# Tomeu7/AO-MARL

Hardware: AMD Instinct MI355X
Metric: env steps/sec (AO frames/sec) (higher is better)
Workload: dtype f32

## Files before the change

ao_marl_amd/csrc/aomarl_capi_composites.hip:

```cpp
const char *aomarl_frame_kernel_name(aomarl_ctx *c) {
  if (!c || !c->fw_variant[0]) return "";
  snprintf(c->fw_name, sizeof(c->fw_name), "k_frame_wave<%d, %d, %s, %s, %s, %s>", c->fw_variant[0], c->fw_variant[1],
           c->fw_variant[2] ? "true" : "false", c->fw_variant[3] ? "true" : "false",
           c->fw_variant[4] ? "true" : "false", c->fw_variant[5] ? "true" : "false");
  return c->fw_name;
}

int aomarl_frame_kernel_time(aomarl_ctx *c, double *total_ms, int *launches) {
  if (!c || !total_ms || !launches) return fail("frame_kernel_time: null argument");
  double tot = 0.0;
  int n = 0;
  for (size_t i = 0; i + 1 < c->fw_ev_used; i += 2) {
    float ms = 0.f;
    HIPCHK(hipEventSynchronize(c->fw_ev[i + 1]));
    HIPCHK(hipEventElapsedTime(&ms, c->fw_ev[i], c->fw_ev[i + 1]));
    tot += ms; n++;
  }
  { const int rrc = fw_ev_rewind(c); if (rrc) return rrc; }
  *total_ms = tot; *launches = n;
  return 0;
}

int aomarl_frame_fused_available(aomarl_ctx *c) {
  return c && c->sys.fused_ok && !c->force_unfused_frame ? 1 : 0;
}

static int frame_fused_impl(aomarl_ctx *c, aomarl_state *st, int b, int n, int flags, void *stream, int slot);

int aomarl_frame_fused(aomarl_ctx *c, aomarl_state *st, int b, int n, int flags, void *stream) {
  return frame_fused_impl(c, st, b, n, flags, stream, -1);
}

static int frame_fused_impl(aomarl_ctx *c, aomarl_state *st, int b, int n, int flags, void *stream, int slot) {
  int rc = check_range(c, st, b, n);
  if (rc) return rc;
  if (slot < 0) {
    rc = atmos_wait_pending(c, stream);
    if (rc) return rc;
    rc = psf_wait_pending(c, stream);
    if (rc) return rc;
  }
  if (!c->sys.fused_ok) return fail("frame_fused: geometry not eligible (see aomarl_frame_fused_available)");
  if (flags & (AOMARL_IMG_FROM_PHASE_BUFFER | AOMARL_IMG_NO_ATMOS | AOMARL_IMG_NO_DMS))
    return fail("frame_fused: FROM_PHASE_BUFFER / NO_ATMOS / NO_DMS are not supported here");
  const bool noise = (flags & AOMARL_IMG_NOISE) && c->sys.noise >= 0.f;
  const bool cube = flags & AOMARL_IMG_WRITE_BINCUBE;
  const bool otf = flags & AOMARL_IMG_DM_FROM_VOLTAGE;
  const int cog = ((flags & AOMARL_IMG_COG) ? 1 : 0) | (c->fused_debug << 8);
  if (otf && !c->sys.otf_ok) return fail("frame_fused: DM_FROM_VOLTAGE needs a separable stack-array lattice (see aomarl_dm_from_voltage_available)");
  if (cube && !st->bincube) return fail("frame_fused: WRITE_BINCUBE needs st->bincube");
  if (!cube && !(cog & 1)) return fail("frame_fused: nothing to produce (neither bincube nor slopes)");
  if (n == 0) return 0;
  hipStream_t s = (hipStream_t)stream;
  Work w = work_layout(c, st->nenv);
  const int W = 2 * c->sys.hw;
  float *TR = st->work + w.TR + (size_t)b * c->sys.pupdiam * W * 2;
  float *TP = st->work + w.TPART + (size_t)b * w.nblk * 4;
  float *PEND = st->work + w.PEND + (size_t)b * (W * W + 4);
  DevState ds = dev_state(st);
  if (w.nblk != c->sys.ntiles) return fail("frame_fused: internal stripe count mismatch");
  const int nb = otf ? c->sys.otf_nb : 1;
  const bool hp = c->dft_mode < 0 ? g_precision != 0 : c->dft_mode == 1;
  const bool qf = FW_QF && otf && !hp && !noise && !cube;
  const bool dma = FW_DMA && otf && (hp || FW_DMA_F32);
  const size_t smm = sizeof(float) * ((qf ? 0 : 2 * 128) + (otf ? 4 * 4 * nb * c->sys.otf_latw : 0)) + FW_SLOT_BYTES(dma) +
                     (dma ? 4 * FWD_WAVE(c->nlayers == 1 ? 1 : 3) : 128) +
                     (qf ? 4 * 16 * (size_t)c->sys.ntiles : 0);
  static const long lds_pad_env = [] { const char *e = getenv("AOMARL_FW_LDS_PAD"); return e ? atol(e) : -1L; }();
  size_t lds_pad = 0;
  if (qf && slot >= 0 && smm >= 40 * 1024) {
    const size_t two_per_cu = (160 * 1024) / 3 + 64;
    lds_pad = lds_pad_env >= 0 ? (size_t)lds_pad_env : (smm < two_per_cu ? (two_per_cu - smm + 63) / 64 * 64 : 0);
    if (smm + lds_pad > 64 * 1024) lds_pad = 0;
  }
  dim3 grid((n + 3) / 4, c->sys.ntiles), blk(256);
#define FW(NL, NB, OTF, NZ, WC, HP) hipExtLaunchKernelGGL((k_frame_wave<NL, NB, OTF, NZ, WC, HP>), grid, blk, smm + lds_pad, s, ev_start, ev_done, 0, c->sys, ds, b, n, cog, TR, TP, w.nblk)
#define FW_H(NL, NB, OTF, NZ, WC) do { if (hp) FW(NL, NB, OTF, NZ, WC, true); else FW(NL, NB, OTF, NZ, WC, false); } while (0)
#define FW_NC(NL, NB, OTF)                                                                     \
  do {                                                                                          \
    if (noise) { if (cube) FW_H(NL, NB, OTF, true, true); else FW_H(NL, NB, OTF, true, false); }     \
    else { if (cube) FW_H(NL, NB, OTF, false, true); else FW_H(NL, NB, OTF, false, false); }         \
  } while (0)
#define FW_L(NL)                                                          \
  do {                                                                    \
    if (!otf) FW_NC(NL, 1, false);                                        \
    else if (nb == 1) FW_NC(NL, 1, true);                                 \
    else FW_NC(NL, 2, true);                                              \
  } while (0)
  const bool timed = !c->capturing && c->time_fw && c->fw_ev_used + 2 <= c->fw_ev.size();
  hipEvent_t ev_start = nullptr, ev_done = nullptr;
  if (c->prefetch_atmos) {
    rc = side_stream(c);
    if (rc) return rc;
    ev_done = slot < 0 ? c->ev_frame : c->pipe.ev_done[slot];
  }
  if (timed) { ev_start = c->fw_ev[c->fw_ev_used]; ev_done = c->fw_ev[c->fw_ev_used + 1]; c->fw_ev_used += 2; }
  hipEvent_t ev_mark = nullptr;
  if (c->capturing) { ev_mark = ev_done; ev_start = nullptr; ev_done = nullptr; }
  if (c->nlayers == 1) FW_L(1); else FW_L(3);
  if (ev_mark) { HIPCHK(hipEventRecord(ev_mark, s)); ev_done = ev_mark; }
  c->frame_marked = false;
  c->fw_variant[0] = c->nlayers == 1 ? 1 : 3; c->fw_variant[1] = otf ? nb : 1; c->fw_variant[2] = otf;
  c->fw_variant[3] = noise; c->fw_variant[4] = cube; c->fw_variant[5] = hp;
  g_arith[hp ? AR_FRAME_SPLIT : AR_FRAME_F32]++;
#undef FW_L
#undef FW_NC
#undef FW_H
#undef FW
  LAUNCHCHK();
  if (slot >= 0) {
    c->pipe.ev_done_cur[slot] = ev_done;
    HIPCHK(hipStreamWaitEvent(c->psf_stream, ev_done, 0));
    if (!c->pipe.cmd_covers_commit)
      HIPCHK(hipStreamWaitEvent(c->psf_stream, c->pipe.ev_commit, 0));
    hipExtLaunchKernelGGL(k_target_finish_mfma, dim3(n), dim3(256), 0, c->psf_stream, nullptr, c->pipe.ev_psf[slot], 0, c->sys, TR,
                          TP, w.nblk, PEND, st->frame + b);
    LAUNCHCHK();
    c->pipe.psf_out[slot] = true;
    return 0;
  }
  if (c->prefetch_atmos) {
    c->ev_frame_cur = ev_done; c->frame_marked = true;
    c->side_joined = false;
    HIPCHK(hipStreamWaitEvent(c->psf_stream, ev_done, 0));
    hipExtLaunchKernelGGL(k_target_finish_mfma, dim3(n), dim3(256), 0, c->psf_stream, nullptr, c->capturing ? nullptr : c->ev_psf, 0,
                          c->sys, TR, TP, w.nblk, PEND, st->frame + b);
    LAUNCHCHK();
    if (c->capturing) HIPCHK(hipEventRecord(c->ev_psf, c->psf_stream));
    c->psf_side = true;
    return 0;
  }
  hipLaunchKernelGGL(k_target_finish_mfma, dim3(n), dim3(256), 0, s, c->sys, TR, TP, w.nblk, PEND, st->frame + b);
  LAUNCHCHK();
  return 0;
}

int aomarl_materialize_dm_shape(aomarl_ctx *c, aomarl_state *st, int b, int n, void *stream) {
  int rc = check_range(c, st, b, n);
  if (rc) return rc;
  if (n == 0) return 0;
  return dm_shape_impl(c, st, b, n, nullptr, false, stream);
}

int aomarl_next_part_one(aomarl_ctx *c, aomarl_state *st, int b, int n, float *accumx, float *accumy,
                         int image_flags, void *stream) {
  int rc = aomarl_move_atmos(c, st, b, n, accumx, accumy, stream);
  if (rc) return rc;
  int fl = (image_flags | AOMARL_IMG_COG | AOMARL_IMG_NOISE) & ~(AOMARL_IMG_NO_ATMOS | AOMARL_IMG_NO_DMS);
  const bool defer = c->defer_dm_shape && aomarl_dm_from_voltage_available(c);
  if (aomarl_frame_fused_available(c) && !(fl & AOMARL_IMG_FROM_PHASE_BUFFER)) {
// ... 146 lines not shown
```

ao_marl_amd/csrc/aomarl_kernels.hip:

```cpp
#include "aomarl_host.h"
#include "aomarl_gemm_p.h"
#include <type_traits>

#define WAVE 64

typedef unsigned u32x4 __attribute__((ext_vector_type(4)));

__device__ __forceinline__ hx2 cvt_h2(float a, float b) {
  return __builtin_bit_cast(hx2, __builtin_amdgcn_cvt_pkrtz(a, b));
}
__device__ __forceinline__ float sub_lo(hx2 h, float a) {
  float r;
  asm("v_fma_mix_f32 %0, %1, -1.0, %2 op_sel_hi:[1,0,0]" : "=v"(r) : "v"(h), "v"(a));
  return r;
}
__device__ __forceinline__ float sub_hi(hx2 h, float a) {
  float r;
  asm("v_fma_mix_f32 %0, %1, -1.0, %2 op_sel:[1,0,0] op_sel_hi:[1,0,0]" : "=v"(r) : "v"(h), "v"(a));
  return r;
}

struct __attribute__((packed, aligned(4))) f4u { float v[4]; };
__device__ __forceinline__ void add4(float acc[4], const float *p) {
  const f4u t = *reinterpret_cast<const f4u *>(p);
// ... 1447 lines not shown
    }
  }
}

struct SpotQf { f32x2 Ml, Mh, Sl, Sh; };

__device__ __forceinline__ SpotQf spot_qf_consts(int lane, const float2 *sTw ) {
  const int q = lane >> 4, c = lane & 15;
  float m[4], sv[4];
#pragma unroll
  for (int s = 0; s < 4; s++) {
    const int d = c - (4 * q + s);
    float a = 0.f, b = 0.f;
    for (int j = 0; j < 16; j++) {
      const float2 w = sTw[((2 * j + 1) * d) & 127];
      a += w.x;
      b = fmaf(0.5f + (float)(j >> 1), w.y, b);
    }
    m[s] = (d != 0 && (d & 1) == 0) ? 0.f : 2.f * a;
    sv[s] = 2.f * b;
  }
  SpotQf k;
  k.Ml = f32x2{m[0], m[1]}; k.Mh = f32x2{m[2], m[3]};
  k.Sl = f32x2{sv[0], sv[1]}; k.Sh = f32x2{sv[2], sv[3]};
  return k;
}

__global__ __launch_bounds__(128) void k_fill_qf_tab(float *__restrict__ tab) {
  __shared__ float2 sTw[128];
  const int tid = threadIdx.x;
  float sn, cs;
  sincospif((float)tid * (1.0f / 64.0f), &sn, &cs);
  sTw[tid] = make_float2(cs, sn);
  __syncthreads();
  if (tid < 64) {
    const SpotQf k = spot_qf_consts(tid, sTw);
    float *o = tab + 8 * tid;
    o[0] = k.Ml.x; o[1] = k.Ml.y; o[2] = k.Mh.x; o[3] = k.Mh.y;
    o[4] = k.Sl.x; o[5] = k.Sl.y; o[6] = k.Sh.x; o[7] = k.Sh.y;
  }
}

typedef unsigned u32x2 __attribute__((ext_vector_type(2)));
__device__ __forceinline__ float swap32_add(float a, float b) {
  const u32x2 t = __builtin_amdgcn_permlane32_swap(__float_as_uint(a), __float_as_uint(b), false, false);
  return __uint_as_float(t[0]) + __uint_as_float(t[1]);
}
__device__ __forceinline__ float swap16_add(float a, float b) {
  const u32x2 t = __builtin_amdgcn_permlane16_swap(__float_as_uint(a), __float_as_uint(b), false, false);
  return __uint_as_float(t[0]) + __uint_as_float(t[1]);
}
__device__ __forceinline__ float spot_qf_moments(const SpotQf &K, const float (&er)[4], const float (&ei)[4], const f32x4 z4) {
  const float Mc[4] = {K.Ml.x, K.Ml.y, K.Mh.x, K.Mh.y}, Sc[4] = {K.Sl.x, K.Sl.y, K.Sh.x, K.Sh.y};
  f32x4 Wr = z4, Wi = z4, V = z4;
#pragma unroll
  for (int s = 0; s < 4; s++) {
    Wr = mfma16(Mc[s], er[s], Wr);
    Wi = mfma16(Mc[s], ei[s], Wi);
    V = mfma16(Sc[s], er[s], V);
  }
  f32x4 G1 = z4, G2 = z4, G3 = z4;
#pragma unroll
  for (int s = 0; s < 4; s++) {
    G1 = mfma16(er[s], Wr[s], G1);
    G2 = mfma16(ei[s], Wr[s], G2);
    G3 = mfma16(ei[s], V[s], G3);
    G1 = mfma16(ei[s], Wi[s], G1);
  }
  PK_GUARD_MFMA();
  f32x2 p0 = pk_mul(pk_lo(G1), K.Ml);
  f32x2 px = pk_mul(pk_lo(G3), K.Ml);
  f32x2 py = pk_mul(pk_lo(G2), K.Sl);
  pk_acc_fma(p0, pk_hi(G1), K.Mh);
  pk_acc_fma(px, pk_hi(G3), K.Mh);
  pk_acc_fma(py, pk_hi(G2), K.Sh);
  const float s0 = p0.x + p0.y, tx = px.x + px.y, ty = py.x + py.y;
  float z = swap16_add(swap32_add(s0, tx), swap32_add(ty, p0.y));
  z += dpp_f<0xB1>(z);
  z += dpp_f<0x4E>(z);
  z += dpp_f<0x141>(z);
  z += dpp_f<0x140>(z);
  return z;
}
__device__ __forceinline__ void qf_slopes(const DevSys &sys, float s0, float tx, float ty, float &sx, float &sy) {
  if (s0 > 0.f) {
    const float inv = 2.f * __builtin_amdgcn_rcpf(s0);
    sx = (fmaf(tx, inv, 7.5f) - sys.cog_offset) * sys.cog_scale;
    sy = (fmaf(-ty, inv, 7.5f) - sys.cog_offset) * sys.cog_scale;
  } else {
    sx = 0.f; sy = 0.f;
  }
}

template <bool NOISE, bool WRITE_CUBE>
__device__ __forceinline__ void spot_finish_v(const DevSys &sys, const DevState &st, int e, int i,
                                              int lane, const float (&v)[2][2][2], int do_cog,
                                              float flux_i) {
  const int q = lane >> 4, c = lane & 15;
  const bool owner = (c & 1) == 0;
  float tot = 0.f;
#pragma unroll
  for (int sy = 0; sy < 2; sy++)
#pragma unroll
    for (int sx = 0; sx < 2; sx++)
#pragma unroll
      for (int h = 0; h < 2; h++) tot += v[sy][sx][h];
  const int Xp = 8 + (c >> 1), Xm = 7 - (c >> 1);
  if (!NOISE && !WRITE_CUBE) {
    const float A0 = (v[0][0][0] + v[0][0][1]) + (v[1][0][0] + v[1][0][1]);
    const float A1 = (v[0][1][0] + v[0][1][1]) + (v[1][1][0] + v[1][1][1]);
    float sx_ = (float)Xp * A0;
    sx_ = fmaf((float)Xm, A1, sx_);
    float sy_ = (float)(8 + 2 * q) * (v[0][0][0] + v[0][1][0]);
    sy_ = fmaf((float)(9 + 2 * q), v[0][0][1] + v[0][1][1], sy_);
    sy_ = fmaf((float)(7 - 2 * q), v[1][0][0] + v[1][1][0], sy_);
    sy_ = fmaf((float)(6 - 2 * q), v[1][0][1] + v[1][1][1], sy_);
    tot = wave_sum_last(A0 + A1);
    sx_ = wave_sum_last(sx_);
    sy_ = wave_sum_last(sy_);
    if (do_cog && lane == 63) {
      float *sl = st.slopes + (long long)e * sys.nslope;
      if (tot > 0.f) {
        const float inv = __builtin_amdgcn_rcpf(tot);
        sl[i] = (sx_ * inv - sys.cog_offset) * sys.cog_scale;
        sl[sys.nvalid + i] = (sy_ * inv - sys.cog_offset) * sys.cog_scale;
      } else {
        sl[i] = 0.f;
        sl[sys.nvalid + i] = 0.f;
      }
    }
    (void)flux_i;
    return;
  }
  tot = wave_sum(owner ? tot : 0.f);
  const float g = tot > 0.f ? sys.nphot * flux_i / tot : 0.f;
  float s0 = 0.f, sx = 0.f, sy = 0.f;
  if (NOISE) {
    const int hh = c & 1;
    const uint32_t sd = st.seeds[e], fr = st.frame[e];
#pragma unroll
    for (int ty_ = 0; ty_ < 2; ty_++)
#pragma unroll
      for (int tx_ = 0; tx_ < 2; tx_++) {
        const int Y = ty_ ? 7 - (2 * q + hh) : 8 + 2 * q + hh, X = tx_ ? Xm : Xp;
        const uint32_t idx = (uint32_t)i * 256u + (uint32_t)(Y * 16 + X);
        const float val = sh_noise((hh ? v[ty_][tx_][1] : v[ty_][tx_][0]) * g, sys.noise, sd, fr, idx);
        if (WRITE_CUBE) st.bincube[((long long)e * sys.nvalid + i) * 256 + Y * 16 + X] = val;
        s0 += val;
        sx += val * (float)X;
        sy += val * (float)Y;
      }
  } else {
#pragma unroll
    for (int ty_ = 0; ty_ < 2; ty_++)
#pragma unroll
      for (int tx_ = 0; tx_ < 2; tx_++)
#pragma unroll
        for (int h = 0; h < 2; h++) {
          const int Y = ty_ ? 7 - (2 * q + h) : 8 + 2 * q + h, X = tx_ ? Xm : Xp;
          const float val = v[ty_][tx_][h] * g;
          if (WRITE_CUBE && owner)
            st.bincube[((long long)e * sys.nvalid + i) * 256 + Y * 16 + X] = val;
          s0 += val;
          sx += val * (float)X;
          sy += val * (float)Y;
        }
// ... 349 lines not shown
          }
      tot = wave_sum(owner ? tot : 0.f);
      sx_ = wave_sum(owner ? sx_ : 0.f);
      sy_ = wave_sum(owner ? sy_ : 0.f);
      if (do_cog && lane == 0) {
        const float inv = tot > 0.f ? 1.0f / tot : 0.f;
        sl[i] = tot > 0.f ? (sx_ * inv - sys.cog_offset) * sys.cog_scale : 0.f;
        sl[sys.nvalid + i] = tot > 0.f ? (sy_ * inv - sys.cog_offset) * sys.cog_scale : 0.f;
      }
    } else {
      tot = wave_sum(owner ? tot : 0.f);
      const float g = tot > 0.f ? sys.nphot * flux_cur / tot : 0.f;
      float s0 = 0.f, sx = 0.f, sy = 0.f;
      if (NOISE) {
        const int hh = c & 1;
        const uint32_t sd = st.seeds[e], fr = st.frame[e];
#pragma unroll
        for (int ty_ = 0; ty_ < 2; ty_++)
#pragma unroll
          for (int tx_ = 0; tx_ < 2; tx_++) {
            const int Y = ty_ ? 7 - (2 * q + hh) : 8 + 2 * q + hh, X = tx_ ? Xm : Xp;
            const uint32_t idx = (uint32_t)i * 256u + (uint32_t)(Y * 16 + X);
            const float val = sh_noise((hh ? v[ty_][tx_][1] : v[ty_][tx_][0]) * g, sys.noise, sd, fr, idx);
            if (WRITE_CUBE) st.bincube[((long long)e * sys.nvalid + i) * 256 + Y * 16 + X] = val;
            s0 += val;
            sx += val * (float)X;
            sy += val * (float)Y;
          }
      } else {
#pragma unroll
        for (int ty_ = 0; ty_ < 2; ty_++)
#pragma unroll
          for (int tx_ = 0; tx_ < 2; tx_++)
#pragma unroll
            for (int h = 0; h < 2; h++) {
              const int Y = ty_ ? 7 - (2 * q + h) : 8 + 2 * q + h, X = tx_ ? Xm : Xp;
              const float val = v[ty_][tx_][h] * g;
              if (WRITE_CUBE && owner)
                st.bincube[((long long)e * sys.nvalid + i) * 256 + Y * 16 + X] = val;
              s0 += val;
              sx += val * (float)X;
              sy += val * (float)Y;
            }
      }
      if (do_cog) {
        s0 = wave_sum((NOISE || owner) ? s0 : 0.f);
        sx = wave_sum((NOISE || owner) ? sx : 0.f);
        sy = wave_sum((NOISE || owner) ? sy : 0.f);
        if (lane == 0) {
          sl[i] = s0 != 0.f ? (sx / s0 - sys.cog_offset) * sys.cog_scale : 0.f;
          sl[sys.nvalid + i] = s0 != 0.f ? (sy / s0 - sys.cog_offset) * sys.cog_scale : 0.f;
        }
      }
    }
    flux_cur = flux_next;
    __builtin_amdgcn_wave_barrier();
  }
}

#define FW_LD 20
#define FW_LIT 0x10000
#define FW_FULL 0x20000
#define FW_SUB 0x40000
__device__ __forceinline__ float sci_rev(float ph, float inv_lambda) { return ph * inv_lambda; }

typedef const int __attribute__((address_space(4))) *const_int_p;
typedef const float __attribute__((address_space(4))) *const_float_p;

template <int NL, bool OTF>
struct FrameRaw {
  float L[NL][4];
  float P[OTF ? 1 : 4], T[8];
  unsigned mrow;
  float F;
  f4u SH;
  float4 CS;
};

template <int NL, int NB, bool OTF, bool NOISE, bool WRITE_CUBE, bool HP>
#ifndef FW_WAVES
#define FW_WAVES 3
#endif
#ifndef FW_QF
#define FW_QF 1
#endif
#ifndef FW_DMA
#define FW_DMA 1
#endif
#ifndef FW_DEPTH
#define FW_DEPTH 2
#endif
#ifndef FW_DMA_F32
#define FW_DMA_F32 1
#endif
#ifndef FW_SLOTS1
#define FW_SLOTS1 0
#endif
#define FW_SLOT_BYTES(dma) ((dma) ? (FW_SLOTS1 ? 2 * 3 * 1024 : 16384) : 16384)
#define FWD_BLK 1152
#define FWD_IMG (2 * 1024 + 128)
#define FWD_WAVE(nl) ((nl) * FWD_IMG)
__global__ __launch_bounds__(256) __attribute__((amdgpu_waves_per_eu(FW_WAVES, FW_WAVES)))
void k_frame_wave(DevSys sys, DevState st, int env_begin,
                                                    int env_count, int do_cog,
                                                    float *__restrict__ TR,
                                                    float *__restrict__ TPART, int nblk) {
  extern __shared__ float smem[];
  const int pd = sys.pupdiam, ntl = sys.ntiles;
  const int tid = threadIdx.x, lane = tid & 63, q = lane >> 4, c = lane & 15;
  const int wv = __builtin_amdgcn_readfirstlane(tid >> 6);
  constexpr bool QF = FW_QF && OTF && !HP && !NOISE && !WRITE_CUBE;
  constexpr bool DMA = FW_DMA && OTF && (HP || FW_DMA_F32);
  float2 *sTw = reinterpret_cast<float2 *>(smem);
  float *lat_all = reinterpret_cast<float *>(sTw + (QF ? 0 : 128));
  float4 *shb = reinterpret_cast<float4 *>(lat_all + 4 * 4 * NB * (OTF ? sys.otf_latw : 0));
  char *dimg = reinterpret_cast<char *>(shb) + FW_SLOT_BYTES(DMA) + (DMA ? wv * FWD_WAVE(NL) : 0);
  float4 *qmom = reinterpret_cast<float4 *>(reinterpret_cast<char *>(shb) + FW_SLOT_BYTES(DMA) + (DMA ? 4 * FWD_WAVE(NL) : 0)) + wv * ntl;
  const int dbg = do_cog >> 8;
  do_cog &= 1;
  const int r = sys.stripe_order[blockIdx.y];
  const int el = 4 * blockIdx.x + wv;
  if constexpr (!QF) {
    if (tid < 128) {
      float sn, cs;
      sincospif((float)tid * (1.0f / 64.0f), &sn, &cs);
      sTw[tid] = make_float2(cs, sn);
    }
    __syncthreads();
  }
  const bool active = el < env_count;
  const int e = env_begin + (active ? el : env_count - 1);
  float Cc[4] = {0.f, 0.f, 0.f, 0.f}, Ss[4] = {0.f, 0.f, 0.f, 0.f};
  if constexpr (!QF) {
#pragma unroll
    for (int s = 0; s < 4; s++) {
      const float2 w = sTw[((4 * q + s) * (2 * c + 1)) & 127];
      Cc[s] = w.x; Ss[s] = w.y;
    }
  }
  SpotTwH twh;
  if (HP) twh = spot_tw_h(Cc, Ss);
  SpotQf qfk;
  if constexpr (QF) {
    const float4 ka = reinterpret_cast<const float4 *>(sys.qf_tab)[2 * lane], kb = reinterpret_cast<const float4 *>(sys.qf_tab)[2 * lane + 1];
    qfk.Ml = f32x2{ka.x, ka.y}; qfk.Mh = f32x2{ka.z, ka.w};
    qfk.Sl = f32x2{kb.x, kb.y}; qfk.Sh = f32x2{kb.z, kb.w};
  }
  unsigned shstep;
  const int y = 16 * r + c;
  const char *layb[NL];
  __amdgpu_buffer_rsrc_t lrs[NL];
  unsigned lpxs[NL], ldim[NL], lvo[NL];
#pragma unroll
  for (int l = 0; l < NL; l++) {
    const DevLayer &L = sys.layers[l];
    layb[l] = reinterpret_cast<const char *>(st.screens + (long long)e * sys.screen_stride + L.screen_off);
    lrs[l] = __builtin_amdgcn_make_buffer_rsrc(const_cast<char *>(layb[l]), 0,
                                               4 * L.dim * (L.dim + RING_PAD), 0x00020000);
    ldim[l] = (unsigned)L.dim;
    int px = L.tox + st.origin[(e * sys.nlayers + l) * 2]; px -= (px >= L.dim) ? L.dim : 0;
    int py = L.toy + st.origin[(e * sys.nlayers + l) * 2 + 1]; py -= (py >= L.dim) ? L.dim : 0;
    lpxs[l] = (unsigned)px;
    unsigned pr = (unsigned)y + (unsigned)py; pr = min(pr, pr - ldim[l]);
    lvo[l] = 4u * (pr * (ldim[l] + RING_PAD) + 4u * (unsigned)q);
  }
  const DevDm &D0 = sys.dms[0], &D1 = sys.dms[1];
  const float *pzt = st.dm_shape + (long long)e * sys.shape_stride + D0.shape_off;
  const float *ttslot = st.dm_shape + (long long)e * sys.shape_stride + D1.shape_off;
  const float c0 = ttslot[0], c1 = ttslot[1];
  const int half = pd / 2;
  const unsigned pvo = 4u * ((unsigned)(y + D0.toy) * (unsigned)D0.dim + (unsigned)D0.tox + 4u * (unsigned)q);
  const unsigned tvo = 32u * ((unsigned)y * (unsigned)(pd >> 2) + (unsigned)q);
  const unsigned mvo = 2u * (unsigned)y * (unsigned)ntl;
  const char *pztb = reinterpret_cast<const char *>(pzt);
  const char *ttb = reinterpret_cast<const char *>(sys.tt_pk);
  const char *mkb = reinterpret_cast<const char *>(sys.tile_mask);
  const bool sh_tt = wv < 2;
  const void *shbase = sh_tt ? static_cast<const void *>(ttb) : (HP ? sys.psf_tw_h : sys.psf_tw_f);
  const __amdgpu_buffer_rsrc_t shrs = __builtin_amdgcn_make_buffer_rsrc(
      const_cast<void *>(shbase), 0, sh_tt ? 8 * pd * pd : ntl * 1024, 0x00020000);
  const unsigned shvo = sh_tt ? tvo + 16u * (unsigned)wv : 16u * (unsigned)lane;
  shstep = sh_tt ? 7u : 10u;
  float pivot;
  {
    float v = OTF ? ttslot[2] : pzt[(half + D0.toy) * D0.dim + half + D0.tox];
    const float2 f = reinterpret_cast<const float2 *>(D1.influ)[(half + D1.toy) * D1.dim + half + D1.tox];
    v += c0 * f.x + c1 * f.y;
#pragma unroll
    for (int l = 0; l < NL; l++) {
      const DevLayer &L = sys.layers[l];
      int py = L.toy + st.origin[(e * sys.nlayers + l) * 2 + 1]; py -= (py >= L.dim) ? L.dim : 0;
      unsigned pyc = (unsigned)(half + py); pyc = min(pyc, pyc - ldim[l]);
      unsigned pxc = (unsigned)half + lpxs[l]; pxc = min(pxc, pxc - ldim[l]);
      v += reinterpret_cast<const float *>(layb[l])[pyc * (ldim[l] + RING_PAD) + pxc];
    }
    pivot = v;
  }
  float Pxr[NB], Pyr[NB];
  const int jm = (c >> 2) + 4 * (c & 3);
  const bool jm_ok = jm < 4 * NB;
// ... 124 lines not shown
        wr[3] = __builtin_amdgcn_cosf(a23.y); wi[3] = __builtin_amdgcn_sinf(a23.y);
        }
        ar[0] = __builtin_amdgcn_cosf(b01.x); ai[0] = __builtin_amdgcn_sinf(b01.x);
        ar[1] = __builtin_amdgcn_cosf(b01.y); ai[1] = __builtin_amdgcn_sinf(b01.y);
        ar[2] = __builtin_amdgcn_cosf(b23.x); ai[2] = __builtin_amdgcn_sinf(b23.x);
        ar[3] = __builtin_amdgcn_cosf(b23.y); ai[3] = __builtin_amdgcn_sinf(b23.y);
        nfull++;
      } else {
        const float ph4[4] = {p01.x, p01.y, p23.x, p23.y};
#pragma unroll
        for (int j = 0; j < 4; j++) {
          const float ph = ph4[j];
          const bool m = (cur.mrow >> (4 * q + j)) & 1u;
          float a_ = ph * wfs_il; a_ -= rintf(a_);
          const float b_ = sci_rev(ph, tar_il);
          wr[j] = m ? __builtin_amdgcn_cosf(a_) : 0.f; wi[j] = m ? __builtin_amdgcn_sinf(a_) : 0.f;
          ar[j] = m ? __builtin_amdgcn_cosf(b_) : 0.f; ai[j] = m ? __builtin_amdgcn_sinf(b_) : 0.f;
          const float d = m ? ph : 0.f;
          sd += d; sd2 += d * d; sm += m ? 1.f : 0.f;
        }
      }
    } else if (info & FW_FULL) {
#pragma unroll
      for (int j = 0; j < 4; j++) {
        float ph = (OTF ? S[j] : cur.P[OTF ? 0 : j]) + (c0 * cur.T[j] + c1 * cur.T[4 + j]);
#pragma unroll
        for (int l = 0; l < NL; l++) ph += cur.L[l][j];
        float a_ = ph * wfs_il; a_ -= rintf(a_);
        const float b_ = sci_rev(ph, tar_il);
        wr[j] = __builtin_amdgcn_cosf(a_); wi[j] = __builtin_amdgcn_sinf(a_);
        ar[j] = __builtin_amdgcn_cosf(b_); ai[j] = __builtin_amdgcn_sinf(b_);
        const float d = ph - pivot;
        sd += d; sd2 += d * d;
      }
      sm += 4.f;
    } else {
#pragma unroll
      for (int j = 0; j < 4; j++) {
        float ph = (OTF ? S[j] : cur.P[OTF ? 0 : j]) + (c0 * cur.T[j] + c1 * cur.T[4 + j]);
#pragma unroll
        for (int l = 0; l < NL; l++) ph += cur.L[l][j];
        const bool m = (cur.mrow >> (4 * q + j)) & 1u;
        float a_ = ph * wfs_il; a_ -= rintf(a_);
        const float b_ = sci_rev(ph, tar_il);
        wr[j] = m ? __builtin_amdgcn_cosf(a_) : 0.f; wi[j] = m ? __builtin_amdgcn_sinf(a_) : 0.f;
        ar[j] = m ? __builtin_amdgcn_cosf(b_) : 0.f; ai[j] = m ? __builtin_amdgcn_sinf(b_) : 0.f;
        const float d = m ? ph - pivot : 0.f;
        sd += d; sd2 += d * d; sm += m ? 1.f : 0.f;
      }
    }
    if constexpr (!NOFETCH) fetch(infon, nxt);
    if (!(dbg & 2)) {
      if constexpr (PK) {
        const f32x2 ar01 = {ar[0], ar[1]}, ar23 = {ar[2], ar[3]}, ai01 = {ai[0], ai[1]}, ai23 = {ai[2], ai[3]};
        PK_GUARD_TRANS();
        const f32x2 sr_ = pk_add(ar01, ar23), si_ = pk_add(ai01, ai23);
        pk_acc_add(R0rp, sr_); pk_acc_add(R0ip, si_);
        PK_END_TO_MFMA();
      } else {
        R0r += (ar[0] + ar[1]) + (ar[2] + ar[3]);
        R0i += (ai[0] + ai[1]) + (ai[2] + ai[3]);
      }
      if (HP) {
        const hx8 csH = __builtin_bit_cast(hx8, csP);
        hx8 arH, arL, aiH, aiL;
        dup_hl(ar[0], ar[1], ar[2], ar[3], arH, arL);
        dup_hl(ai[0], ai[1], ai[2], ai[3], aiH, aiL);
        PA = mfma_h(arH, csH, PA); PA = mfma_h(arL, csH, PA);
        PB = mfma_h(aiH, csH, PB); PB = mfma_h(aiL, csH, PB);
      } else {
        PA = mfma16(ar[0], csP.x, PA); PB = mfma16(ai[0], csP.x, PB);
        PA = mfma16(ar[1], csP.y, PA); PB = mfma16(ai[1], csP.y, PB);
        PA = mfma16(ar[2], csP.z, PA); PB = mfma16(ai[2], csP.z, PB);
        PA = mfma16(ar[3], csP.w, PA); PB = mfma16(ai[3], csP.w, PB);
      }
    }
    if ((info & FW_SUB) && !(dbg & 1)) {
      if (HP) {
        float v[2][2][2];
        spot_dft_h_v(twh, wr, wi, Z4, v);
        spot_finish_v<NOISE, WRITE_CUBE>(sys, st, e, info & 0xFFFF, lane, v, do_cog, flux_i);
      } else if (!NOISE && !WRITE_CUBE) {
        if constexpr (QF) {
          const float z = spot_qf_moments(qfk, wr, wi, Z4);
          if (c == 0 && q < 3) reinterpret_cast<float *>(qmom + t)[q] = z;
        } else if constexpr (PK) spot_cog_f32_pk(sys, st, e, info & 0xFFFF, lane, Cc, Ss, wr, wi, do_cog, Z4);
        else spot_cog_f32(sys, st, e, info & 0xFFFF, lane, Cc, Ss, wr, wi, do_cog, Z4);
      } else {
        spot_core<NOISE, WRITE_CUBE>(sys, st, e, info & 0xFFFF, lane, Cc, Ss, wr, wi, do_cog, flux_i, Z4);
      }
    }
  };

  if constexpr (DMA) {
    const std::integral_constant<int, 1> dm;
    const int np = sys.pair_count[r];
    const const_int_p pinfo = (const_int_p)(unsigned long long)(sys.pair_info + r * (2 * ((ntl + 1) / 2 + 2)));
    const int rr = lane >> 3, kk = (lane & 7) ^ rr;
    unsigned dvo[NL][2];
#pragma unroll
    for (int l = 0; l < NL; l++) {
      const DevLayer &L = sys.layers[l];
      int py = L.toy + st.origin[(e * sys.nlayers + l) * 2 + 1]; py -= (py >= L.dim) ? L.dim : 0;
#pragma unroll
      for (int b = 0; b < 2; b++) {
        unsigned pr = (unsigned)(16 * r + 8 * b + rr) + (unsigned)py; pr = min(pr, pr - ldim[l]);
        dvo[l][b] = 4u * (pr * (ldim[l] + RING_PAD)) + 16u * (unsigned)kk;
      }
    }
    const int bc = c >> 3, rc = c & 7;
    const char *rdp[2];
#pragma unroll
    for (int h = 0; h < 2; h++) rdp[h] = dimg + bc * FWD_BLK + 16 * (rc * 8 + ((4 * h + q) ^ rc));
    const unsigned dimg_lds = (unsigned)(unsigned long long)dimg;
    FrameRaw<NL, OTF> A, B;
    unsigned mrA, mrB;
    float fA, fB;
    const unsigned shb_lds = (unsigned)(unsigned long long)shb + 1024u * (unsigned)wv;
    auto dma16 = [&](unsigned vo, __amdgpu_buffer_rsrc_t rs, unsigned lds_addr, unsigned so) {
      unsigned keep;
      asm volatile("s_mov_b32 %0, m0\n\ts_mov_b32 m0, %3\n\ts_nop 0\n\tbuffer_load_dwordx4 %1, %2, %4 offen lds\n\ts_mov_b32 m0, %0"
                   : "=&s"(keep) : "v"(vo), "s"(rs), "s"(lds_addr), "s"(so) : "memory");
    };
    auto issue_shared = [&](int ia, int ib, int par) {
      const int ta = (ia >> 24) & 0x7F, tb = (ib >> 24) & 0x7F;
      if (FW_SLOTS1) {
        if (wv < 3) {
          dma16(shvo, shrs, shb_lds, (unsigned)ta << shstep);
          dma16(shvo, shrs, shb_lds + 3072u, (unsigned)tb << shstep);
        }
      } else {
        dma16(shvo, shrs, shb_lds + (unsigned)par * 8192u, (unsigned)ta << shstep);
        dma16(shvo, shrs, shb_lds + (unsigned)par * 8192u + 4096u, (unsigned)tb << shstep);
      }
    };
    auto issue = [&](int ia, int ib) {
      const int ta = (ia >> 24) & 0x7F, tb = (ib >> 24) & 0x7F;
      mrA = *reinterpret_cast<const uint16_t *>(mkb + 2u * (unsigned)ta + mvo);
      mrB = *reinterpret_cast<const uint16_t *>(mkb + 2u * (unsigned)tb + mvo);
      fA = cflux[ia & 0xFFFF];
      fB = cflux[ib & 0xFFFF];
#pragma unroll
      for (int l = 0; l < NL; l++) {
        unsigned sx = 16u * (unsigned)(ta & ~1) + lpxs[l]; sx -= (sx >= ldim[l]) ? ldim[l] : 0u;
        const unsigned so = 4u * sx;
#pragma unroll
        for (int b = 0; b < 2; b++) dma16(dvo[l][b], lrs[l], dimg_lds + l * FWD_IMG + b * FWD_BLK, so);
      }
    };
    int ia = pinfo[0], ib = pinfo[1];
    if (np > 0) { issue_shared(ia, ib, 0); issue(ia, ib); }
    for (int k = 0; k < np; k++) {
      const int ja = pinfo[2 * k + 2], jb = pinfo[2 * k + 3];
      asm volatile("s_waitcnt vmcnt(0)" ::: "memory");
#pragma unroll
      for (int l = 0; l < NL; l++) {
        const float4 va = *reinterpret_cast<const float4 *>(rdp[0] + l * FWD_IMG);
        const float4 vb = *reinterpret_cast<const float4 *>(rdp[1] + l * FWD_IMG);
        A.L[l][0] = va.x; A.L[l][1] = va.y; A.L[l][2] = va.z; A.L[l][3] = va.w;
        B.L[l][0] = vb.x; B.L[l][1] = vb.y; B.L[l][2] = vb.z; B.L[l][3] = vb.w;
      }
      A.mrow = mrA; A.F = fA; B.mrow = mrB; B.F = fB;
      asm volatile("s_waitcnt lgkmcnt(0)" ::: "memory");
      if (FW_SLOTS1) {
        if (k + 1 < np) issue(ja, jb);
        __syncthreads();
        float4 *slots = shb;
// ... 884 lines not shown
```

Before: 538,800.

## Compute spot moments via LDS transpose and six MFMAs in quadratic-form path

```diff
diff --git a/ao_marl_amd/csrc/aomarl_capi_composites.hip b/ao_marl_amd/csrc/aomarl_capi_composites.hip
--- a/ao_marl_amd/csrc/aomarl_capi_composites.hip
+++ b/ao_marl_amd/csrc/aomarl_capi_composites.hip
@@ -65,7 +65,7 @@
   const bool dma = FW_DMA && otf && (hp || FW_DMA_F32);
   const size_t smm = sizeof(float) * ((qf ? 0 : 2 * 128) + (otf ? 4 * 4 * nb * c->sys.otf_latw : 0)) + FW_SLOT_BYTES(dma) +
                      (dma ? 4 * FWD_WAVE(c->nlayers == 1 ? 1 : 3) : 128) +
-                     (qf ? 4 * 16 * (size_t)c->sys.ntiles : 0);
+                     (qf ? 4 * 16 * (size_t)c->sys.ntiles + (FW_QF == 2 ? 4 * 1024 : 0) : 0);
   static const long lds_pad_env = [] { const char *e = getenv("AOMARL_FW_LDS_PAD"); return e ? atol(e) : -1L; }();
   size_t lds_pad = 0;
   if (qf && slot >= 0 && smm >= 40 * 1024) {
diff --git a/ao_marl_amd/csrc/aomarl_kernels.hip b/ao_marl_amd/csrc/aomarl_kernels.hip
--- a/ao_marl_amd/csrc/aomarl_kernels.hip
+++ b/ao_marl_amd/csrc/aomarl_kernels.hip
@@ -1553,6 +1553,52 @@
   z += dpp_f<0x140>(z);
   return z;
 }
+
+__device__ __forceinline__ int qf_swz(int k) { return (((k ^ (k >> 1)) & 1) << 1) | (k >> 1); }
+__device__ __forceinline__ f32x4 qf_transpose(float *qw, const f32x4 *qr, const float (&e)[4]) {
+  __builtin_amdgcn_wave_barrier();
+#pragma unroll
+  for (int s = 0; s < 4; s++) qw[16 * s] = e[s];
+  __builtin_amdgcn_wave_barrier();
+  return *qr;
+}
+__device__ __forceinline__ float spot_qf_moments6(const SpotQf &K, const float (&er)[4], const float (&ei)[4],
+                                                  float *qw, const f32x4 *qr, const f32x4 z4) {
+  const float Mc[4] = {K.Ml.x, K.Ml.y, K.Mh.x, K.Mh.y}, Sc[4] = {K.Sl.x, K.Sl.y, K.Sh.x, K.Sh.y};
+  f32x4 etr = qf_transpose(qw, qr, er);
+  f32x4 eti = qf_transpose(qw, qr, ei);
+  __builtin_amdgcn_sched_barrier(0);
+  f32x4 ErM = z4, EiM = z4, EiSt = z4, MEr = z4, MEi = z4, SEi = z4;
+#pragma unroll
+  for (int s = 0; s < 4; s++) {
+    ErM = mfma16(er[s], Mc[s], ErM);
+    EiM = mfma16(ei[s], Mc[s], EiM);
+    EiSt = mfma16(ei[s], Sc[s], EiSt);
+  }
+  asm volatile("" : "+v"(ErM), "+v"(EiM), "+v"(EiSt), "+v"(etr), "+v"(eti));
+#pragma unroll
+  for (int s = 0; s < 4; s++) {
+    MEr = mfma16(Mc[s], etr[s], MEr);
+    MEi = mfma16(Mc[s], eti[s], MEi);
+    SEi = mfma16(Sc[s], eti[s], SEi);
+  }
+  PK_GUARD_MFMA();
+  f32x2 p0 = pk_mul(pk_lo(MEr), pk_lo(ErM));
+  f32x2 px = pk_mul(pk_lo(EiSt), pk_lo(MEr));
+  f32x2 py = pk_mul(pk_lo(SEi), pk_lo(ErM));
+  pk_acc_fma(p0, pk_hi(MEr), pk_hi(ErM));
+  pk_acc_fma(px, pk_hi(EiSt), pk_hi(MEr));
+  pk_acc_fma(py, pk_hi(SEi), pk_hi(ErM));
+  pk_acc_fma(p0, pk_lo(MEi), pk_lo(EiM));
+  pk_acc_fma(p0, pk_hi(MEi), pk_hi(EiM));
+  const float s0 = p0.x + p0.y, tx = -px.x - px.y, ty = py.x + py.y;
+  float z = swap16_add(swap32_add(s0, tx), swap32_add(ty, p0.y));
+  z += dpp_f<0xB1>(z);
+  z += dpp_f<0x4E>(z);
+  z += dpp_f<0x141>(z);
+  z += dpp_f<0x140>(z);
+  return z;
+}
 __device__ __forceinline__ void qf_slopes(const DevSys &sys, float s0, float tx, float ty, float &sx, float &sy) {
   if (s0 > 0.f) {
     const float inv = 2.f * __builtin_amdgcn_rcpf(s0);
@@ -2068,7 +2114,7 @@
 #define FW_WAVES 3
 #endif
 #ifndef FW_QF
-#define FW_QF 1
+#define FW_QF 2
 #endif
 #ifndef FW_DMA
 #define FW_DMA 1
@@ -2101,7 +2147,11 @@
   float *lat_all = reinterpret_cast<float *>(sTw + (QF ? 0 : 128));
   float4 *shb = reinterpret_cast<float4 *>(lat_all + 4 * 4 * NB * (OTF ? sys.otf_latw : 0));
   char *dimg = reinterpret_cast<char *>(shb) + FW_SLOT_BYTES(DMA) + (DMA ? wv * FWD_WAVE(NL) : 0);
-  float4 *qmom = reinterpret_cast<float4 *>(reinterpret_cast<char *>(shb) + FW_SLOT_BYTES(DMA) + (DMA ? 4 * FWD_WAVE(NL) : 0)) + wv * ntl;
+  float4 *qmom_all = reinterpret_cast<float4 *>(reinterpret_cast<char *>(shb) + FW_SLOT_BYTES(DMA) + (DMA ? 4 * FWD_WAVE(NL) : 0));
+  float4 *qmom = qmom_all + wv * ntl;
+  float *qtb = reinterpret_cast<float *>(qmom_all + 4 * ntl) + 256 * wv;
+  float *qtw = qtb + 64 * q + 4 * ((c >> 2) ^ qf_swz(q)) + (c & 3);
+  const f32x4 *qtr = reinterpret_cast<const f32x4 *>(qtb + 16 * c + 4 * (q ^ qf_swz(c >> 2)));
   const int dbg = do_cog >> 8;
   do_cog &= 1;
   const int r = sys.stripe_order[blockIdx.y];
@@ -2392,7 +2442,7 @@
         spot_finish_v<NOISE, WRITE_CUBE>(sys, st, e, info & 0xFFFF, lane, v, do_cog, flux_i);
       } else if (!NOISE && !WRITE_CUBE) {
         if constexpr (QF) {
-          const float z = spot_qf_moments(qfk, wr, wi, Z4);
+          const float z = FW_QF == 2 ? spot_qf_moments6(qfk, wr, wi, qtw, qtr, Z4) : spot_qf_moments(qfk, wr, wi, Z4);
           if (c == 0 && q < 3) reinterpret_cast<float *>(qmom + t)[q] = z;
         } else if constexpr (PK) spot_cog_f32_pk(sys, st, e, info & 0xFFFF, lane, Cc, Ss, wr, wi, do_cog, Z4);
         else spot_cog_f32(sys, st, e, info & 0xFFFF, lane, Cc, Ss, wr, wi, do_cog, Z4);
```

After: 545,500, median of 6. +1.2%, better.
